# sailist/emotion-recognition-in-conversation

Measured on AMD Instinct MI355X. Metric: utterances/sec training step, COGMEN IEMOCAP-6 atv, higher is better.
Workload: dtype bf16

## Files before the change

emotion-recognition-in-conversation_amd/capi.py:

```python
import ctypes as C
import os
import re
import subprocess

import torch

_HERE = os.path.dirname(os.path.abspath(__file__))
LIB_PATH = os.environ.get("ERC_LIB_PATH") or os.path.join(_HERE, "lib", "libercgraft.so")
CSRC = os.path.join(_HERE, "csrc")
HEADER = os.path.join(os.path.dirname(_HERE), "include", "ercgraft.h")


class ErcGraftError(RuntimeError):
    pass


_CTYPES = {"int": C.c_int, "int32_t": C.c_int, "int64_t": C.c_int64, "uint64_t": C.c_uint64, "float": C.c_float}


def _ctype(decl, proto, ret=False):
    t = " ".join(decl.replace("*", " * ").split())
    if ret and t == "const char *":
        return C.c_char_p
    if "*" in t:
# ... 940 lines not shown
        _call("erc_dgcn_tail", *args)
    else:
        _call("erc_dgcn_tail_cap", *args, n_dev, label_rows)


def dgcn_tail_eval(slabs, n_slabs, slab_stride, rgcn_bias, g, window, W_rel, b_rel, W_root, W1, b1, W2, b2, labels, n_classes,
                   n_rows, Xc, ldx, cm, logits=None, n_dev=None, label_rows=None):
    if cm.dtype != torch.int64 or cm.numel() != n_classes * n_classes or not cm.is_contiguous():
        raise ErcGraftError("dgcn_tail_eval: cm must be a contiguous int64 [%d, %d] tensor" % (n_classes, n_classes))
    _call("erc_dgcn_tail_eval", slabs, n_slabs, int(slab_stride), rgcn_bias, g["in_ptr"], g["in_src"], window, W_rel, b_rel, W_root,
          W1, b1, W2, b2, labels, label_rows, n_classes, n_rows, n_dev, Xc, ldx, cm, logits)


def head_ce_stats_floats(n_rows):
    return int(lib().erc_head_ce_stats_floats(n_rows))


def head_ce(Z, ldz, F, Cn, n_rows, W, bias, labels, weight, mask_scale, logits, ldl, dlogits, lddl, dZ, lddz, stats, n_dev=None):
    args = (Z, ldz, F, Cn, n_rows, W, bias, labels, weight, float(mask_scale), logits, ldl, dlogits, lddl, dZ, lddz, stats)
    if n_dev is None:
        _call("erc_head_ce", *args)
    else:
        _call("erc_head_ce_cap", *args, n_dev)


def cim_meta(lengths, B, T, n_cap, node_off, node_row):
    _call("erc_cim_meta", lengths, B, T, n_cap, node_off, node_row)


def gru_scan_fwd(GX, W_hhT, b_hh, lengths, node_off, B, T, rows, Hout, Hdrop, drop_p, rng, rng_stream, gates, ghn, Hprev):
    _call("erc_gru_scan_fwd", GX, W_hhT, b_hh, lengths, node_off, B, T, rows, Hout, Hdrop, drop_p, rng, rng_stream, gates, ghn,
          Hprev)


def gru_scan_bwd(W_hh, lengths, node_off, B, T, rows, gates, ghn, Hprev, dH, drop_p, rng, rng_stream, dGX, dGH):
    _call("erc_gru_scan_bwd", W_hh, lengths, node_off, B, T, rows, gates, ghn, Hprev, dH, drop_p, rng, rng_stream, dGX, dGH)


def cim_max_t():
    return int(lib().erc_cim_max_t())


def cim_attn_fwd(merged, node_off, B, T, Pbuf):
    _call("erc_cim_attn_fwd", merged, node_off, B, T, Pbuf)


def cim_attn_bwd(merged, dmerged, node_off, B, T, Pbuf, mask_scale):
    _call("erc_cim_attn_bwd", merged, dmerged, node_off, B, T, Pbuf, mask_scale)


def ce_bce_multitask(logits, ld, Cn, n_rows, labels, emo_label, lde, w_ce, w_bce, grad_scale, dlogits, lddl, stats):
    if labels.dtype != torch.int64 or emo_label.dtype != torch.int64:
        raise ErcGraftError("ce_bce_multitask: label and emo_label must be int64")
    if labels.numel() < n_rows or emo_label.dim() != 2 or emo_label.shape[0] < n_rows or emo_label.shape[1] < 7 \
            or emo_label.stride(1) != 1 or logits.numel() < (n_rows - 1) * ld + Cn + 7:
        raise ErcGraftError("ce_bce_multitask: operands smaller than %d rows (label %s, emo_label %s)"
                            % (n_rows, tuple(labels.shape), tuple(emo_label.shape)))
    _call("erc_ce_bce_multitask", logits, ld, Cn, n_rows, labels, emo_label, lde, w_ce, w_bce, grad_scale, dlogits, lddl,
          stats)


def dgcnv2_max_t():
    return int(lib().erc_dgcnv2_max_t())


def dgcnv2_meta(onehot, S, lengths, B, T, n_cap, spk, node_row):
    _call("erc_dgcnv2_meta", onehot, S, lengths, B, T, n_cap, spk, node_row)


def dgcnv2_edge_att_fwd(S, ldS, g, B, T, wp, wf, norm):
    _call("erc_dgcnv2_edge_att_fwd", S, ldS, g["node_off"], B, T, wp, wf, g["out_ptr"], g["out_dst"], g["out_eid"], norm)


def dgcnv2_edge_att_bwd(S, ldS, g, B, T, wp, wf, dnorm, dS, dn_parts=1, dn_stride=0):
    _call("erc_dgcnv2_edge_att_bwd", S, ldS, g["node_off"], B, T, wp, wf, g["out_ptr"], g["out_dst"], g["out_eid"], dnorm,
          dn_parts, dn_stride, dS)


def match_att_fwd(E, lde, Q, ldq, node_off, B, T, F, A, lda, P, TH):
    _call("erc_match_att_fwd", E, lde, Q, ldq, node_off, B, T, F, A, lda, P, TH)


def match_att_bwd(E, lde, Q, ldq, dA, ldda, node_off, B, T, F, P, TH, DZ, dQ, lddq, dE, ldde, n_cap=0):
    args = (E, lde, Q, ldq, dA, ldda, node_off, B, T, F, P, TH, DZ, dQ, lddq, dE, ldde)
    if n_cap:
        _call("erc_match_att_bwd_cap", *args, n_cap)
    else:
        _call("erc_match_att_bwd", *args)


DIALOGRNN_SAVE = {"gates_g": (0, 450), "ghn_g": (450, 150), "g_prev": (600, 150), "g": (750, 150), "g_drop": (900, 150),
                  "c": (1050, 150), "gates_p": (1200, 450), "ghn_p": (1650, 150), "q_prev": (1800, 150), "q": (1950, 150),
                  "q_drop": (2100, 150), "gates_e": (2250, 300), "ghn_e": (2550, 100), "e_prev": (2650, 100), "e": (2750, 100),
                  "e_drop": (2850, 100)}
DIALOGRNN_DREC = {"dgh_g": (0, 450), "dgh_p": (450, 450), "dgi_e": (900, 300), "dgh_e": (1200, 300)}
DIALOGRNN_DREC_ROW = 1500
DIALOGRNN_GXW = 1050


def dialogrnn_max_t():
    return int(lib().erc_dialogrnn_max_t())


def dialogrnn_wt_floats():
    return int(lib().erc_dialogrnn_wt_floats())


def dialogrnn_save_floats(N, B, T):
    return int(lib().erc_dialogrnn_save_floats(N, B, T))


def dialogrnn_planes(buf, N, layout):
    return {k: buf[o * 2 * N:(o + w) * 2 * N].view(2, N, w) for k, (o, w) in layout.items()}


def dialogrnn_alpha(save, N, B, T):
    o = 2950 * 2 * N
    return save[o:o + 2 * B * T * T].view(2, B, T, T)


def dialogrnn_offsets(offs):
    if len(offs) != 20:
        raise ErcGraftError("dialogrnn: 20 parameter offsets expected, got %d" % len(offs))
    return (C.c_int64 * 20)(*[int(o) for o in offs])


def dialogrnn_meta(onehot, S, lengths, B, T, n_cap, node_off, node_row, node_spk):
    _call("erc_dialogrnn_meta", onehot, S, lengths, B, T, n_cap, node_off, node_row, node_spk)


def dialogrnn_pack(params, offs, D_m, WT):
    _call("erc_dialogrnn_pack", params, C.addressof(offs), D_m, WT)


def dialogrnn_scan_fwd(GX, ldgx, WT, params, offs, D_m, node_off, node_spk, B, T, S, N, drop_p, drop_rec, rng, rng_stream,
                       emotions, lde, save):
    _call("erc_dialogrnn_scan_fwd", GX, ldgx, WT, params, C.addressof(offs), D_m, node_off, node_spk, B, T, S, N, float(drop_p),
          float(drop_rec), rng, rng_stream, emotions, lde, save)


def dialogrnn_scan_bwd(GX, ldgx, WT, params, offs, D_m, node_off, node_spk, B, T, S, N, drop_p, drop_rec, rng, rng_stream, save,
                       dEmo, ldde, dGX, lddgx, dREC):
    _call("erc_dialogrnn_scan_bwd", GX, ldgx, WT, params, C.addressof(offs), D_m, node_off, node_spk, B, T, S, N, float(drop_p),
          float(drop_rec), rng, rng_stream, save, dEmo, ldde, dGX, lddgx, dREC)


def bcrnn_meta_cap(lengths, desc, store_label, zero_store_row, B, T, n_cap, node_off, node_row, pad_node, x_row, label_out, counts):
    _call("erc_bcrnn_meta_cap", lengths, desc, store_label, zero_store_row, B, T, n_cap, node_off, node_row, pad_node, x_row,
          label_out, counts)


def log_softmax_rows(x, ldx, Cn, n_rows, y, ldy):
    _call("erc_log_softmax_rows", x, ldx, Cn, n_rows, y, ldy)
```

emotion-recognition-in-conversation_amd/engine.py:

```python
import math
import os

import torch

from . import capi

ALIGN = 64


class WorkspaceCache:

    def __init__(self, maxsize=None):
        import collections
        self.maxsize = int(os.environ.get("ERC_WS_CACHE", 4)) if maxsize is None else maxsize
        self._d = collections.OrderedDict()
        self.last = None

    def get(self, key, make):
        ws = self._d.get(key)
        if ws is None:
            ws = make()
            self._d[key] = ws
            while len(self._d) > self.maxsize:
                victim = next((k for k in self._d if k != key), None)
# ... 410 lines not shown
        dev = flat.device
        self.state = torch.zeros(4 + 512, dtype=torch.int64, device=dev)
        self.state[2] = seed
        self.gnorm = torch.zeros(1, dtype=torch.float32, device=dev)
        self.norm_ws = torch.zeros(1024, dtype=torch.float32, device=dev)
        self.shadow = None
        self.shadow_table = None
        self.skip_flag = None

    def set_step(self, step):
        self.state[0] = int(step)
        self.state[4:] = int(step)

    @property
    def rng_state(self):
        return self.state[1:3]

    def enable_p2p(self, group=None):
        import torch.distributed as dist
        if os.environ.get("ERC_DP_P2P", "0") != "1" or not (dist.is_available() and dist.is_initialized()) or \
                dist.get_world_size(group) < 2 or self.clip_norm > 0 or self.flat.numel > P2PExchange.MAX_PARAMS:
            return False
        try:
            self.flat.p2p = P2PExchange(self.flat, group)
        except P2PUnavailable as exc:
            import sys
            print("ERC_DP_P2P=1: %s -- keeping the RCCL all-reduce" % exc, file=sys.stderr)
            return False
        self.skip_flag = self.flat.health
        return True

    def step(self, grad_scale=1.0):
        f = self.flat
        if getattr(f, "p2p", None) is not None:
            capi.adam_step_p2p(f.data, f.grad, f.exp_avg, f.exp_avg_sq, f.numel, self.lr, self.betas[0], self.betas[1], self.eps,
                               self.weight_decay, self.decoupled, grad_scale, self.state, self.shadow_table, f.p2p.desc)
            return
        if self.clip_norm > 0:
            capi.grad_norm(f.grad, f.numel, grad_scale, self.gnorm, self.norm_ws)
        if self.shadow_table is not None:
            capi.adam_step_tab(f.data, f.grad, f.exp_avg, f.exp_avg_sq, f.numel, self.lr, self.betas[0], self.betas[1],
                               self.eps, self.weight_decay, self.decoupled, grad_scale, self.clip_norm,
                               self.gnorm if self.clip_norm > 0 else None, self.state, self.shadow_table,
                               skip_flag=self.skip_flag)
            return
        capi.adam_step(f.data, f.grad, f.exp_avg, f.exp_avg_sq, f.numel, self.lr, self.betas[0], self.betas[1],
                       self.eps, self.weight_decay, self.decoupled, grad_scale, self.clip_norm,
                       self.gnorm if self.clip_norm > 0 else None, self.state,
                       *(self.shadow if self.shadow is not None else (None, 0, 0)), skip_flag=self.skip_flag)


class P2PUnavailable(RuntimeError):
    """the fused gradient exchange cannot be set up on this node (every rank raises it together)"""


class P2PExchange:

    MAX_PARAMS = 512 * 1024

    def __init__(self, flat, group=None):
        import ctypes as C
        import torch.distributed as dist
        self.world, self.rank = dist.get_world_size(group), dist.get_rank(group)
        if self.world > 8 or flat.numel > self.MAX_PARAMS or flat.numel % 4:
            raise capi.ErcGraftError("P2P gradient exchange: world <= 8 and <= %d parameters (this module: %d)" % (
                self.MAX_PARAMS, flat.numel))
        self.n_pad = flat.numel
        self._mine, self._peers = [], []
        try:
            self._mine = [capi.p2p_alloc(2 * self.n_pad * 4), capi.p2p_alloc(self.world * 512 * 4)]
            mine = (self._mine[0][1], self._mine[1][1])
        except capi.ErcGraftError as exc:
            mine = None
            self.alloc_error = str(exc)
        handles = [None] * self.world
        dist.all_gather_object(handles, mine, group=group)
        if any(h is None for h in handles):
            self.close()
            raise P2PUnavailable("rank(s) %s could not allocate uncached peer-visible memory" % [r for r, h in enumerate(handles) if h is None])
        self.allocation = "hipDeviceMallocUncached"
        x = capi.ErcP2P()
        x.world, x.rank, x.spin_limit, x.n_pad = self.world, self.rank, int(os.environ.get("ERC_P2P_SPIN", 0)), self.n_pad
        for r in range(self.world):
            if r == self.rank:
                x.pub[r], x.flags[r] = self._mine[0][0], self._mine[1][0]
            else:
                pp, pf = capi.p2p_open(handles[r][0]), capi.p2p_open(handles[r][1])
                self._peers += [pp, pf]
                x.pub[r], x.flags[r] = pp, pf
        self.epoch = torch.zeros(512, dtype=torch.int64, device=flat.device)
        x.epoch, x.health = self.epoch.data_ptr(), flat.health.data_ptr()
        self.desc, self.flat = x, flat
        dist.barrier(group=group)

    def close(self):
        for p in self._peers:
            capi.p2p_close(p)
        self._peers = []
        for p, _ in self._mine:
            capi.p2p_free(p)
        self._mine = []


def all_reduce_grads(flat, always=False):
    import torch.distributed as dist
    if dist.is_available() and dist.is_initialized() and (dist.get_world_size() > 1 or always):
        if getattr(flat, "p2p", None) is not None:
            return 1.0 / dist.get_world_size()
        dist.all_reduce(flat.grad_full)
        return 1.0 / dist.get_world_size()
    return 1.0


class SideStream:

    def __init__(self, enabled=None):
        if enabled is None:
            import os
            enabled = os.environ.get("ERC_SIDE_STREAM", "0") == "1"
        self.enabled = enabled and torch.cuda.is_available()
        self.stream = torch.cuda.Stream() if self.enabled else None
        self._dirty = False

    def fork(self):
        return _Fork(self)

    def join(self):
        if self.enabled and self._dirty:
            ev = torch.cuda.Event()
            ev.record(self.stream)
            torch.cuda.current_stream().wait_event(ev)
            self._dirty = False


class _Fork:
    def __init__(self, side):
        self.side = side

    def __enter__(self):
        if self.side.enabled:
            ev = torch.cuda.Event()
            ev.record()
            self.side.stream.wait_event(ev)
            self.ctx = torch.cuda.stream(self.side.stream)
            self.ctx.__enter__()
            self.side._dirty = True

    def __exit__(self, *exc):
        if self.side.enabled:
            self.ctx.__exit__(*exc)
        return False


class GraphedStep:

    def __init__(self, fn, warmup=2, steps=1):
        self.fn = fn
        side = torch.cuda.Stream()
        side.wait_stream(torch.cuda.current_stream())
        with torch.cuda.stream(side):
            for _ in range(warmup):
                self.out = fn()
        torch.cuda.current_stream().wait_stream(side)
        torch.cuda.synchronize()
        self.graph = torch.cuda.CUDAGraph()
        with torch.cuda.graph(self.graph):
            for _ in range(steps):
                self.out = fn()
        self.warmup_steps, self.steps = warmup, steps

    def __call__(self):
        self.graph.replay()
        return self.out
```

emotion-recognition-in-conversation_amd/trainer.py:

```python
import contextlib
import dataclasses
import json
import os
import sys
import time

import numpy as np
import torch
from torch.utils.data import DataLoader

from . import capi
from .capacity import node_capacity
from .collate import ERCCollate
from .synthetic import make_dialogues, make_mosei_dialogues


def fix_seed(seed):
    import random
    random.seed(seed)
    np.random.seed(seed)
    torch.manual_seed(seed)
    if torch.cuda.is_available():
        torch.cuda.manual_seed_all(seed)


class ListDataset(torch.utils.data.Dataset):

    def __init__(self, dialogs):
        self.dialogs = dialogs

    def __len__(self):
        return len(self.dialogs)

    def __getitem__(self, i):
        return [self.dialogs[i]]


class StoreLoader:

    def __init__(self, store, batch_size, shuffle, seed):
        self.store, self.batch_size, self.shuffle = store, batch_size, shuffle
        self.gen = torch.Generator().manual_seed(seed)

    def __len__(self):
        return -(-len(self.store) // self.batch_size)

    def __iter__(self):
        n = len(self.store)
        order = torch.randperm(n, generator=self.gen) if self.shuffle else torch.arange(n)
        for i in range(0, n, self.batch_size):
            yield self.store.batch(order[i:i + self.batch_size])


def shard_dialogues(dialogs, rank, world):
    n = len(dialogs)
    if world <= 1 or n == 0:
        return list(dialogs)
    total = -(-n // world) * world
    idx = [i % n for i in range(total)]
    return [dialogs[i] for i in idx[rank::world]]


def load_dialogues(params, rank=0, world=1):
    if not params.get("synthetic", True):
        from .datasets import read_dialogues
        roots = params.get("data_root", None)
        train = read_dialogues(params.dataset, "train", roots)
        return shard_dialogues(train, rank, world), read_dialogues(params.dataset, "test", roots)
    meld, mosei = "meld" in params.dataset, "mosei" in params.dataset
    lo, hi = (1, 33) if meld else (1, 98) if mosei else (20, 110)
    lo, hi = int(params.get("syn_min_len", lo)), int(params.get("syn_max_len", hi))
    if mosei:
        mk = lambda n, seed: make_mosei_dialogues(n, params.dims(), min_len=lo, max_len=hi, seed=seed)
        return mk(params.n_train, params.seed + 1000 * rank), mk(params.n_test, params.seed + 7)
    mk = lambda n, seed: make_dialogues(n, params.dims(), n_speakers=params.n_speakers, n_classes=params.n_classes,
                                        min_len=lo, max_len=hi, seed=seed)
    return mk(params.n_train, params.seed + 1000 * rank), mk(params.n_test, params.seed + 7)


def make_loaders(params, rank=0, world=1, device=None):
    train_d, test_d = load_dialogues(params, rank, world)
    if params.get("device_collate", False):
        from .datasets import DeviceDialogueStore
        dt = torch.bfloat16 if params.compute == "bf16" else torch.float32
        return (StoreLoader(DeviceDialogueStore(train_d, params, device, dt), params.train.batch_size, True, params.seed + rank),
                StoreLoader(DeviceDialogueStore(test_d, params, device, dt), params.test.batch_size, False, 0))
    train, test = ListDataset(train_d), ListDataset(test_d)
    collate = ERCCollate(params)
    gen = torch.Generator().manual_seed(params.seed + rank)
    tl = DataLoader(train, batch_size=params.train.batch_size, shuffle=True, collate_fn=collate,
                    num_workers=params.train.get("num_workers", 0) or 0, generator=gen)
    el = DataLoader(test, batch_size=params.test.batch_size, shuffle=False, collate_fn=collate, num_workers=0)
    return tl, el


def longest_dialogue(loader):
    if isinstance(loader, StoreLoader):
        return int(loader.store.lengths.max())
    return max(len(d["label"]) for d in loader.dataset.dialogs)


def bucket_t_cap(loader, world, device):
    t = longest_dialogue(loader)
    if world > 1:
        import torch.distributed as dist
        v = torch.tensor([t], dtype=torch.int64, device=device)
        dist.all_reduce(v, op=dist.ReduceOp.MAX)
        t = int(v.item())
    return t


def first_batch(loader):
    if isinstance(loader, StoreLoader):
        return loader.store.batch(torch.arange(min(loader.batch_size, len(loader.store))))
    n = min(loader.batch_size, len(loader.dataset))
    return loader.collate_fn([loader.dataset[i] for i in range(n)])


class FixedBatches:

    def __init__(self, loader, trainer, seed):
        self.batches = [(int(b["label"].shape[0]), trainer.prepare_batch(b)) for b in loader]
        self.gen = torch.Generator().manual_seed(seed)

    def __len__(self):
        return len(self.batches)

    def __iter__(self):
        for i in torch.randperm(len(self.batches), generator=self.gen).tolist():
            yield i, self.batches[i]


def batch_table(lengths, offsets, order, B):
    n = len(order)
    steps = -(-n // B)
    flat = np.zeros((2, steps * B), dtype=np.int32)
    flat[0, :n], flat[1, :n] = lengths[order], offsets[order]
    return np.concatenate([flat[0].reshape(steps, B), flat[1].reshape(steps, B)], axis=1)


@contextlib.contextmanager
def dynamic_n(model, on=True):
    if on:
        model.dynamic_n = True
    try:
        yield
    finally:
        if on:
            model.dynamic_n = False


@dataclasses.dataclass
class GraphEntry:
    static: dict
    fill: object
    capacity: bool
    seen: int = 0
    graph: object = None
    out: object = None
    workspace: object = None


class StepGraphs:

    def __init__(self, trainer, maxsize=16, capture=True):
        import collections
        self.trainer, self.maxsize = trainer, maxsize
        self.capture = capture
        self.cache = collections.OrderedDict()
        self.replays = self.eager = self.captures = 0
        self.capture_failed = False
        self.lazy = True

    def _capture(self, fn):
        torch.cuda.synchronize()
        g = torch.cuda.CUDAGraph()
        with torch.cuda.graph(g):
            out = fn()
        return g, out

    def _sync(self):
        torch.cuda.synchronize()

    @staticmethod
    def shape_key(batch):
        return tuple((k, tuple(v.shape), str(v.dtype)) for k, v in sorted(batch.items()) if torch.is_tensor(v)) + \
            tuple((k, v) for k, v in sorted(batch.items()) if isinstance(v, int))

    @staticmethod
    def _copy_in(static, batch):
        for k, v in batch.items():
            if torch.is_tensor(v):
                static[k].copy_(v, non_blocking=True)

    def _eager_then_capture(self, ent, capture=True, must=False):
        tr = self.trainer
        with dynamic_n(tr.model, ent.capacity):
            stats = tr.train_step(ent.static)
            if not capture:
                return stats
            try:
                ent.graph, ent.out = self._capture(lambda: tr.train_step(ent.static))
            except Exception as exc:
                if must:
                    raise
                print(json.dumps({"graph_replay": "capture failed, staying eager", "error": str(exc)[:200]}), file=sys.stderr)
                self.capture_failed = True
                return stats
        ent.workspace = getattr(tr.model, "_last_ws", None)
        self.captures += 1
        return stats

    def precapture(self, probe):
        tr = self.trainer
        flat, model = tr.model.flat, tr.model
        opt = getattr(tr, "optim", None)
        saved = {k: v.clone() for k, v in model.state_dict().items() if "running_" in k or "num_batches" in k}
        snap = [(t, t.clone()) for t in (getattr(flat, n, None) for n in ("data", "exp_avg", "exp_avg_sq", "grad_full")) if t is not None]
        if opt is not None and getattr(opt, "state", None) is not None:
            snap.append((opt.state, opt.state.clone()))
        if getattr(flat, "p2p", None) is not None:
            snap.append((flat.p2p.epoch, flat.p2p.epoch.clone()))
        for key, make, fill, synth in tr.all_capacity_buckets(probe):
            ent = self.cache[key] = GraphEntry(make(), fill, True, seen=1)
            synth(ent.static)
            self._eager_then_capture(ent, must=True)
        self._sync()
        with torch.no_grad():
            for t, keep in snap:
                t.copy_(keep)
            sd = model.state_dict()
            for k, v in saved.items():
                sd[k].copy_(v)
        flat.health.zero_()
        flat.events.zero_()
        if getattr(model, "shadows", None) is not None:
            model.refresh_shadows()
        self.maxsize = max(self.maxsize, len(self.cache) + 2)

    def step(self, batch, key=None, resident=False):
        bucket = None
        if key is not None:
            key = (key, )
        else:
            bucket = self.trainer.capacity_bucket(batch) if hasattr(self.trainer, "capacity_bucket") else None
            key = bucket[0] if bucket is not None else self.shape_key(batch)
        ent = self.cache.get(key)
        if ent is None and not self.lazy:
            self.eager += 1
            return self.trainer.train_step(batch)
        if ent is None:
            if bucket is not None:
                static, fill = bucket[1](), bucket[2]
            else:
                static = batch if resident else {k: (v.clone() if torch.is_tensor(v) else v) for k, v in batch.items()}
                fill = None if resident else self._copy_in
            ent = self.cache[key] = GraphEntry(static, fill, bucket is not None)
            while len(self.cache) > self.maxsize:
                self.cache.popitem(last=False)
        else:
            self.cache.move_to_end(key)
        ent.seen += 1
        if ent.fill is not None and (ent.graph is not None or ent.seen > 1 or ent.capacity):
            ent.fill(ent.static, batch)
        if ent.graph is not None:
            self.replays += 1
            ent.graph.replay()
            return ent.out
        self.eager += 1
        return self._eager_then_capture(ent, capture=self.capture and not self.capture_failed and
                                        (ent.capacity or ent.seen >= 2 or resident))


class ResidentLoop:

    N_BUCKET = 128

    def __init__(self, trainer, store, batch_size, capture=True):
        self.trainer, self.store, self.B = trainer, store, int(batch_size)
        self.T = int(store.lengths.max())
        named = getattr(trainer, "RESIDENT_N_BUCKET", None)
        if named:
            self.N_BUCKET = max(1, min(int(named), self.B * self.T))
        self.cur_desc = torch.zeros(2 * self.B, dtype=torch.int32, device=store.device)
        self.graphs, self.capture = {}, capture
        self.replays = self.eager = self.captures = 0

    def _capture(self, fn):
        torch.cuda.synchronize()
        g = torch.cuda.CUDAGraph()
        with torch.cuda.graph(g):
            fn()
        return g

    def _caps_of(self, counts):
        return [node_capacity(c, self.N_BUCKET, self.B * self.T) for c in counts]

    def _visit(self, cap):
        ent = self.graphs.get(cap)
        batch = ent[1] if ent is not None else self._batch(cap)
        if batch is None:
            raise capi.ErcGraftError("%s: the trainer offers no resident batch of capacity %d" % (type(self).__name__, cap))
        ws = self._step(batch)
        self.eager += 1
        graph = None
        if self.capture:
            graph = self._capture(lambda: self._step(batch))
            self.captures += 1
        self.graphs[cap] = (graph, batch, ws)

    def _steps(self, table_dev, caps):
        cur_desc, graphs = self.cur_desc, self.graphs
        for s, cap in enumerate(caps):
            cur_desc.copy_(table_dev[s], non_blocking=True)
            ent = graphs.get(cap)
            if ent is not None and ent[0] is not None:
                ent[0].replay()
                self.replays += 1
                continue
            self._visit(cap)


class ResidentEpochs(ResidentLoop):

    def __init__(self, trainer, store, batch_size, seed, capture=True):
        super().__init__(trainer, store, batch_size, capture)
        self.gen = torch.Generator().manual_seed(seed)
        self.acc = torch.zeros(4, dtype=torch.float64, device=store.device)
        self._lens32, self._offs32 = store.lengths.to(torch.int32).numpy(), store.offsets[:-1].to(torch.int32).numpy()
        self._ahead = []

    def plan(self, n_epochs):
        n, B = len(self.store), self.B
        tabs = np.zeros((n_epochs, -(-n // B), 2 * B), dtype=np.int32)
        for e in range(n_epochs):
            tabs[e] = batch_table(self._lens32, self._offs32, torch.randperm(n, generator=self.gen).numpy(), B)
        dev = torch.from_numpy(tabs).to(self.store.device)
        for e in range(n_epochs):
            counts = tabs[e, :, :B].sum(1).tolist()
            self._ahead.append((sum(counts), self._caps_of(counts), dev[e]))

    def supported(self):
        lens = sorted((int(v) for v in self.store.lengths.tolist()), reverse=True)
        worst = self._caps_of([sum(lens[:self.B])])[0]
        return all(self._batch(cap) is not None for cap in sorted({self.N_BUCKET, max(worst, self.N_BUCKET)}))

    def _batch(self, cap):
        return self.trainer.resident_batch(self.store, self.cur_desc, self.B, self.T, cap)

    def _step(self, batch):
        self.acc.add_(self.trainer.train_step(batch)[:4])
        return getattr(self.trainer.model, "_last_ws", None)

    def epoch(self):
        if not self._ahead:
            self.plan(1)
        n_utt, caps, table_dev = self._ahead.pop(0)
        with dynamic_n(self.trainer.model):
            self._steps(table_dev, caps)
        return n_utt, len(caps)


class ResidentEval(ResidentLoop):

    def __init__(self, trainer, store, batch_size, capture=True, n_classes=None):
        super().__init__(trainer, store, batch_size, capture)
        self.table = batch_table(store.lengths.to(torch.int32).numpy(), store.offsets[:-1].to(torch.int32).numpy(),
                                 np.arange(len(store)), self.B)
        self.steps = len(self.table)
        self.counts = self.table[:, :self.B].sum(1).tolist()
        self.caps = self._caps_of(self.counts)
        self.table_dev = torch.from_numpy(self.table).to(store.device)
        C = int(n_classes if n_classes is not None else trainer.params.n_classes)
        self.cm = torch.zeros(C, C, dtype=torch.int64, device=store.device)

    def supported(self):
        return all(self._batch(cap) is not None for cap in sorted(set(self.caps)))

    def _batch(self, cap):
        return self.trainer.resident_eval_batch(self.store, self.cur_desc, self.B, self.T, cap)

    def _step(self, batch):
        return self.trainer.resident_eval_step(batch, self.cm)

    def epoch(self):
        self.cm.zero_()
        self._steps(self.table_dev, self.caps)
        return self.cm.cpu()


def report_from_cm(cm):
    cm = np.asarray(cm, dtype=np.int64)
    n = int(cm.sum())
    tp, sup, prd = np.diag(cm).astype(np.float64), cm.sum(1).astype(np.float64), cm.sum(0).astype(np.float64)
    div = lambda a, b: np.divide(a, b, out=np.zeros_like(a), where=b > 0)
    rec, pre, f1 = div(tp, sup), div(tp, prd), div(2.0 * tp, sup + prd)
    weighted = lambda v: float((v * sup).sum() / n) if n else 0.0
    acc = float(tp.sum() / n) if n else 0.0
    seen = (sup > 0) | (prd > 0)
    return {
        "cm": cm.tolist(),
        "acc": acc,
        "wa": float(rec[sup > 0].mean()) if n else 0.0,
        "pre": weighted(pre),
        "rec": weighted(rec),
        "f1": weighted(f1),
        "mif1": acc,
        "maf1": float(f1[seen].mean()) if n else 0.0,
    }


def classification_report(true, pred, n_classes):
    from sklearn import metrics
    return {
        "cm": metrics.confusion_matrix(true, pred, labels=range(n_classes)).tolist(),
        "acc": metrics.accuracy_score(true, pred),
        "wa": metrics.balanced_accuracy_score(true, pred),
        "pre": metrics.precision_score(true, pred, average="weighted", zero_division=0),
        "rec": metrics.recall_score(true, pred, average="weighted", zero_division=0),
        "f1": metrics.f1_score(true, pred, average="weighted", zero_division=0),
        "mif1": metrics.f1_score(true, pred, average="micro", zero_division=0),
        "maf1": metrics.f1_score(true, pred, average="macro", zero_division=0),
    }


def weighted_accuracy(y_true, y_pred):
    y_true, y_pred = np.asarray(y_true), np.asarray(y_pred)
    P = int((y_true == 1).sum())
    N = len(y_true) - P
    if P == 0 or N == 0:
        return None
    TP = int(((y_true == 1) & (y_pred == 1)).sum())
    TN = int(((y_true == 0) & (y_pred == 0)).sum())
    return (1.0 * TP * (N / (1.0 * P)) + TN) / (2.0 * N)


def multiemo_report(true_multi, prob_multi, thresh=0.5):
    from sklearn import metrics
    true_multi, pred = np.asarray(true_multi), (np.asarray(prob_multi) > thresh).astype(int)
    acc, f1, wa = [], [], []
    for i in range(true_multi.shape[1]):
        col = pred[:, i]
        acc.append(float(metrics.accuracy_score(true_multi[:, i], col)))
        f1.append(float(metrics.precision_recall_fscore_support(true_multi[:, i], col, average="weighted", zero_division=0)[2]))
        wa.append(weighted_accuracy(true_multi[:, i], col))
    defined = [w for w in wa if w is not None]
# ... 192 lines not shown
```

include/ercgraft.h:

```cpp
#ifndef ERCGRAFT_H
#define ERCGRAFT_H

#include <stdint.h>

#ifdef __cplusplus
extern "C" {
#endif

#define ERC_ABI_VERSION 3

#define ERC_OK 0
#define ERC_E_ARG (-1)
#define ERC_E_LAUNCH (-2)

int erc_abi_version(void);
const char* erc_last_error(void);

int erc_window_graph_build(const int64_t* lengths, const int64_t* speakers, int64_t spk_sb, int64_t spk_st,
                           int B, int T, int wp, int wf, int n_speakers, int n_cap, int e_cap,
                           int32_t* node_off, int32_t* node_row, int32_t* node_spk,
                           int32_t* in_ptr, int32_t* in_src, int32_t* in_typ,
                           int32_t* out_ptr, int32_t* out_dst, int32_t* out_typ, int32_t* out_eid,
                           int64_t* edge_index, int64_t* edge_type, int32_t* counts, void* stream);
int erc_window_graph_build_desc(const int64_t* lengths, const int64_t* speakers, int64_t spk_sb, int64_t spk_st,
// ... 404 lines not shown
int erc_transpose_batched(const float* in, int nb, int rows, int cols, float* out, void* stream);
int erc_csr_sum(const float* x, int ldx, int F, int N, const int32_t* ptr, const int32_t* idx, float* out, int ldo,
                int accumulate, void* stream);

int erc_dgcn_tail_max_rows(void);
int erc_dgcn_tail_set_stamps(uint64_t* stamps);
int erc_dgcn_tail_max_window(void);
int64_t erc_dgcn_tail_stats_floats(int n_rows);
int erc_dgcn_tail(const float* slabs, int n_slabs, int64_t slab_stride, const float* rgcn_bias, const int32_t* in_ptr,
                  const int32_t* in_src, int window, const float* W_rel, const float* b_rel, const float* W_root,
                  const float* W1, const float* b1, const float* W2, const float* b2, const int64_t* labels,
                  const float* weight, int n_classes, int n_rows, float drop_p, const uint64_t* rng, float* Xc, int ldx,
                  float* Hc, float* AGG, float* Zc, float* logits, float* dlogits, float* dZc, float* dXc, int lddx,
                  float* dAGG, float* dHc, float* stats, void* stream);
int erc_dgcn_tail_cap(const float* slabs, int n_slabs, int64_t slab_stride, const float* rgcn_bias, const int32_t* in_ptr,
                      const int32_t* in_src, int window, const float* W_rel, const float* b_rel, const float* W_root,
                      const float* W1, const float* b1, const float* W2, const float* b2, const int64_t* labels,
                      const float* weight, int n_classes, int n_rows, float drop_p, const uint64_t* rng, float* Xc, int ldx,
                      float* Hc, float* AGG, float* Zc, float* logits, float* dlogits, float* dZc, float* dXc, int lddx,
                      float* dAGG, float* dHc, float* stats, const int32_t* n_dev, const int32_t* label_rows, void* stream);

int erc_dgcn_tail_eval(const float* slabs, int n_slabs, int64_t slab_stride, const float* rgcn_bias, const int32_t* in_ptr,
                       const int32_t* in_src, int window, const float* W_rel, const float* b_rel, const float* W_root,
                       const float* W1, const float* b1, const float* W2, const float* b2, const int64_t* labels,
                       const int32_t* label_rows, int n_classes, int n_rows, const int32_t* n_dev, const float* Xc, int ldx,
                       int64_t* cm, float* logits, void* stream);

int erc_gemm_f32_grouped(int form, const float* A, int lda, const float* B, int ldb, float* C, int ldc,
                         int N_or_K, const int32_t* node_off, int n_dialogues, int n_mod, int n_nodes,
                         int max_len, int pitch, int accumulate, int act, const float* aux, int ldaux,
                         float act_scale,
                         const float* cross, int planes, int64_t a_plane, int64_t b_plane, int split, int64_t c_slab,
                         void* stream);
int erc_gemm_f32_planes(const float* A, int lda, int64_t a_plane, const float* B, int ldb, int64_t b_plane, float* C,
                        int ldc, int M, int N, int K, int planes, int split_k, int64_t c_slab, int accumulate,
                        void* stream);
int erc_mm_meta(const int64_t* lengths, const float* qmask, int64_t q_st, int64_t q_sb, int n_speakers, int B,
                int32_t* node_off, int32_t* node_row, int32_t* node_dlg, int32_t* node_spk, void* stream);
int erc_mm_flatten(const float* src, int lds, const int32_t* row_map, const float* emb, const int32_t* spk, int N,
                   float* dst, int ldd, void* stream);
int64_t erc_mm_emb_grad_ws_floats(int n_speakers);
int erc_mm_emb_grad(const float* dl, int ld, const int32_t* spk, int N, int n_speakers, float* demb, float* ws,
                    void* stream);
int erc_mm_row_normalize(const float* x, int R, float* xhat, float* inv, void* stream);
int erc_mm_row_normalize_bwd(const float* xhat, const float* inv, const float* dxhat, int R, float* dx, void* stream);
int erc_mm_adj_finish(const float* COS, const float* xhat, const int32_t* node_off, int B, int M, int N, int P,
                      float* ADJ, float* CR, float* CCOS, float* DEG, void* stream);
int erc_mm_adj_finish_bwd(const float* COS, const float* CCOS, const float* DEG, const float* dADJ, const float* dCR,
                          const int32_t* node_off, int B, int M, int N, int P, float* G, float* GC, float* DD,
                          void* stream);
int erc_mm_cross_apply(const float* CR, const float* h, int ldh, const int32_t* node_dlg, const int32_t* node_off,
                       int M, int N, int P, float* out, int ldo, void* stream);
int erc_mm_cross_grad(const float* dhi, int ldd, const float* h, int ldh, const int32_t* node_dlg,
                      const int32_t* node_off, int M, int N, int P, float* dCR, int planes, int64_t d_plane,
                      int64_t h_plane, void* stream);
int erc_gcnii_combine_fwd(const float* G, const float* hi, const float* h0, int64_t n, float theta, float alpha,
                          float drop_p, const uint64_t* rng_state, uint64_t rng_stream, float* hd, void* stream);
int erc_gcnii_combine_bwd(const float* d_hd, const float* hd, int64_t n, float theta, float alpha, float keep_scale,
                          int plain, float* dG, float* dhi, float* dh0, int F, int ld_d, void* stream);
int erc_gcnii_layer_fwd(const float* hih0, int lda, const float* W, int ldw, float theta, float alpha, float drop_p,
                        const uint64_t* rng_state, uint64_t rng_stream, float* hd, int ldo, int rows, int F, void* stream);
int erc_dropout_fwd(const float* x, int64_t n, float drop_p, const uint64_t* rng_state, uint64_t rng_stream, float* y,
                    void* stream);
int erc_mm_regroup_fwd(const float* xd, const float* hl, int M, int N, float drop_p, const uint64_t* rng_state,
                       uint64_t rng_stream, float* FE, void* stream);
int erc_mm_regroup_bwd(const float* dFE, const float* FE, int M, int N, float keep_scale, float* d_xd, float* d_h,
                       void* stream);
int erc_axpy_mask(const float* x, const float* mask, int64_t n, float scale, int accumulate, float* y, void* stream);
int erc_mm_meta_cap(const int64_t* lengths, const float* qmask, int64_t q_st, int64_t q_sb, int n_speakers, const int32_t* desc,
                    const int64_t* store_spk, const int64_t* store_label, int zero_store_row, int B, int T, int n_cap,
                    int32_t* node_off, int32_t* node_row, int32_t* node_pad, int32_t* node_dlg, int32_t* node_spk,
                    int32_t* pad_node, int32_t* x_row, int64_t* label_out, int32_t* counts, void* stream);
int erc_mm_flatten_cap(const float* src, int lds, const int32_t* row_map, const float* emb, const int32_t* spk, int n_cap,
                       const int32_t* n_dev, float* dst, int ldd, void* stream);
int erc_mm_emb_grad_cap(const float* dl, int ld, const int32_t* spk, int n_cap, const int32_t* n_dev, int n_speakers, float* demb,
                        float* ws, void* stream);
int erc_mm_row_normalize_cap(const float* x, int n_mod, int n_cap, const int32_t* n_dev, float* xhat, float* inv, void* stream);
int erc_mm_row_normalize_bwd_cap(const float* xhat, const float* inv, const float* dxhat, int n_mod, int n_cap,
                                 const int32_t* n_dev, float* dx, void* stream);
int erc_mm_cross_apply_cap(const float* CR, const float* h, int ldh, const int32_t* node_dlg, const int32_t* node_off, int M,
                           int n_cap, const int32_t* n_dev, int P, float* out, int ldo, void* stream);
int erc_mm_cross_grad_cap(const float* dhi, int ldd, const float* h, int ldh, const int32_t* node_dlg, const int32_t* node_off,
                          int M, int n_cap, const int32_t* n_dev, int P, float* dCR, int planes, int64_t d_plane,
                          int64_t h_plane, void* stream);
int erc_gcnii_combine_bwd_cap(const float* d_hd, const float* hd, int n_mod, int n_cap, const int32_t* n_dev, float theta,
                              float alpha, float keep_scale, int plain, float* dG, float* dhi, float* dh0, int F, int ld_d,
                              void* stream);
int erc_dropout_fwd_cap(const float* x, int n_mod, int n_cap, const int32_t* n_dev, int row_w, float drop_p,
                        const uint64_t* rng_state, uint64_t rng_stream, float* y, void* stream);
int erc_mm_regroup_fwd_cap(const float* xd, const float* hl, int M, int n_cap, const int32_t* n_dev, float drop_p,
                           const uint64_t* rng_state, uint64_t rng_stream, float* FE, void* stream);
int erc_mm_regroup_bwd_cap(const float* dFE, const float* FE, int M, int n_cap, const int32_t* n_dev, float keep_scale,
                           float* d_xd, float* d_h, void* stream);
int erc_axpy_mask_cap(const float* x, const float* mask, int n_mod, int n_cap, const int32_t* n_dev, int row_w, float scale,
                      int accumulate, float* y, void* stream);
int erc_mm_zero_tail(float* buf, int64_t ld, int width, int n_mod, int n_cap, const int32_t* n_dev, void* stream);


int erc_cim_meta(const int64_t* lengths, int B, int T, int n_cap, int32_t* node_off, int32_t* node_row, void* stream);
int erc_gru_scan_fwd(const float* GX, const float* W_hhT, const float* b_hh, const int64_t* lengths, const int32_t* node_off,
                     int B, int T, int64_t rows, float* Hout, float* Hdrop, float drop_p, const uint64_t* rng_state,
                     uint64_t rng_stream, float* gates, float* ghn, float* Hprev, void* stream);
int erc_gru_scan_bwd(const float* W_hh, const int64_t* lengths, const int32_t* node_off, int B, int T, int64_t rows,
                     const float* gates, const float* ghn, const float* Hprev, const float* dH, float drop_p,
                     const uint64_t* rng_state, uint64_t rng_stream, float* dGX, float* dGH, void* stream);
int erc_cim_max_t(void);
int erc_cim_attn_fwd(float* merged, const int32_t* node_off, int B, int T, float* Pbuf, void* stream);
int erc_cim_attn_bwd(const float* merged, float* dmerged, const int32_t* node_off, int B, int T, const float* Pbuf,
                     float mask_scale, void* stream);
int erc_ce_bce_multitask(const float* logits, int ld, int C, int n_rows, const int64_t* label, const int64_t* emo_label,
                         int lde, float w_ce, float w_bce, float grad_scale, float* dlogits, int lddl, float* stats,
                         void* stream);

int erc_dgcnv2_max_t(void);
int erc_dgcnv2_meta(const float* onehot, int S, const int64_t* lengths, int B, int T, int n_cap, int64_t* spk,
                    int32_t* node_row, void* stream);
int erc_dgcnv2_edge_att_fwd(const float* S, int ldS, const int32_t* node_off, int B, int T, int wp, int wf,
                            const int32_t* out_ptr, const int32_t* out_dst, const int32_t* out_eid, float* norm, void* stream);
int erc_dgcnv2_edge_att_bwd(const float* S, int ldS, const int32_t* node_off, int B, int T, int wp, int wf,
                            const int32_t* out_ptr, const int32_t* out_dst, const int32_t* out_eid, const float* dnorm,
                            int dn_parts, int64_t dn_stride, float* dS, void* stream);


int erc_match_att_fwd(const float* E, int lde, const float* Q, int ldq, const int32_t* node_off, int B, int T, int F, float* A,
                      int lda, float* P, float* TH, void* stream);
int erc_match_att_bwd(const float* E, int lde, const float* Q, int ldq, const float* dA, int ldda, const int32_t* node_off,
                      int B, int T, int F, const float* P, const float* TH, float* DZ, float* dQ, int lddq, float* dE, int ldde,
                      void* stream);
int erc_match_att_bwd_cap(const float* E, int lde, const float* Q, int ldq, const float* dA, int ldda, const int32_t* node_off,
                          int B, int T, int F, const float* P, const float* TH, float* DZ, float* dQ, int lddq, float* dE,
                          int ldde, int n_cap, void* stream);


int erc_dialogrnn_max_t(void);
int64_t erc_dialogrnn_wt_floats(void);
int64_t erc_dialogrnn_save_floats(int64_t N, int B, int T);
int erc_dialogrnn_meta(const float* onehot, int S, const int64_t* lengths, int B, int T, int n_cap, int32_t* node_off,
                       int32_t* node_row, int32_t* node_spk, void* stream);
int erc_dialogrnn_pack(const float* params, const int64_t* offs_host, int D_m, float* WT, void* stream);
int erc_dialogrnn_scan_fwd(const float* GX, int ldgx, const float* WT, const float* params, const int64_t* offs_host, int D_m,
                           const int32_t* node_off, const int32_t* node_spk, int B, int T, int S, int64_t N, float drop_p,
                           float drop_rec, const uint64_t* rng_state, uint64_t rng_stream, float* emotions, int lde,
                           float* save, void* stream);
int erc_dialogrnn_scan_bwd(const float* GX, int ldgx, const float* WT, const float* params, const int64_t* offs_host, int D_m,
                           const int32_t* node_off, const int32_t* node_spk, int B, int T, int S, int64_t N, float drop_p,
                           float drop_rec, const uint64_t* rng_state, uint64_t rng_stream, const float* save,
                           const float* dEmo, int ldde, float* dGX, int lddgx, float* dREC, void* stream);
int erc_bcrnn_meta_cap(const int64_t* lengths, const int32_t* desc, const int64_t* store_label, int zero_store_row, int B, int T,
                       int n_cap, int32_t* node_off, int32_t* node_row, int32_t* pad_node, int32_t* x_row, int64_t* label_out,
                       int32_t* counts, void* stream);
int erc_log_softmax_rows(const float* x, int ldx, int C, int n_rows, float* y, int ldy, void* stream);


int erc_test_poison_lds(int32_t* sink, void* stream);

#ifdef __cplusplus
}
#endif
#endif
```

Measured before the change: 21.38 million.

## Replay captured training steps as direct kernel launches instead of HIP graph replay

Adds a HIP-side chain builder that reads a captured step graph, checks that it is a single linear path of this library's kernel nodes, and records each node's function, grid, block, shared-memory size and argument pointers. In the default auto mode, captured steps then replay by issuing those kernels with hipLaunchKernel in order, and fall back to hipGraph replay when the graph does not qualify. The intent is to avoid HIP graph launch overhead in a launch-bound training step. In exchange, it keeps the raw graph alive so the argument pointers stay valid, pays host-side per-kernel launch cost, and only applies to purely linear graphs.

```diff
diff --git a/emotion-recognition-in-conversation_amd/capi.py b/emotion-recognition-in-conversation_amd/capi.py
--- a/emotion-recognition-in-conversation_amd/capi.py
+++ b/emotion-recognition-in-conversation_amd/capi.py
@@ -1116,3 +1116,31 @@
 
 def log_softmax_rows(x, ldx, Cn, n_rows, y, ldy):
     _call("erc_log_softmax_rows", x, ldx, Cn, n_rows, y, ldy)
+
+
+def chain_order(n_nodes, edges):
+    ne = len(edges)
+    fr, to = (C.c_int32 * max(1, ne))(*[e[0] for e in edges]), (C.c_int32 * max(1, ne))(*[e[1] for e in edges])
+    order = (C.c_int32 * max(1, n_nodes))()
+    _call("erc_chain_order", n_nodes, ne, C.addressof(fr), C.addressof(to), C.addressof(order))
+    return list(order)[:n_nodes]
+
+
+def chain_build(raw_graph):
+    handle = int(lib().erc_chain_build(raw_graph))
+    return (handle, None) if handle else (0, lib().erc_last_error().decode())
+
+
+def chain_len(chain):
+    n = int(lib().erc_chain_len(chain))
+    if n < 0:
+        _check(n, "erc_chain_len")
+    return n
+
+
+def chain_run(chain):
+    _check(lib().erc_chain_run(chain, stream()), "erc_chain_run")
+
+
+def chain_free(chain):
+    _check(lib().erc_chain_free(chain), "erc_chain_free")
diff --git a/emotion-recognition-in-conversation_amd/csrc/launch_chain.hip b/emotion-recognition-in-conversation_amd/csrc/launch_chain.hip
--- /dev/null
+++ b/emotion-recognition-in-conversation_amd/csrc/launch_chain.hip
@@ -0,0 +1,144 @@
+#include <dlfcn.h>
+
+#include <vector>
+
+#include "erc_common.h"
+
+extern "C" int erc_chain_order(int n_nodes, int n_edges, const int32_t* from_host, const int32_t* to_host, int32_t* order_host) {
+    ERC_REQUIRE(n_nodes > 0 && order_host != nullptr, "chain_order: n_nodes=%d (need >= 1 and an output array)", n_nodes);
+    ERC_REQUIRE(n_edges == n_nodes - 1, "chain_order: %d nodes with %d edges are not one path", n_nodes, n_edges);
+    ERC_REQUIRE(n_edges == 0 || (from_host != nullptr && to_host != nullptr), "chain_order: null edge list");
+    std::vector<int32_t> next(n_nodes, -1), pred(n_nodes, -1);
+    for (int e = 0; e < n_edges; ++e) {
+        const int32_t a = from_host[e], b = to_host[e];
+        ERC_REQUIRE(a >= 0 && a < n_nodes && b >= 0 && b < n_nodes && a != b, "chain_order: edge %d (%d -> %d) out of range", e, a, b);
+        ERC_REQUIRE(next[a] < 0, "chain_order: node %d has two successors (a fork)", a);
+        ERC_REQUIRE(pred[b] < 0, "chain_order: node %d has two predecessors (a join)", b);
+        next[a] = b;
+        pred[b] = a;
+    }
+    int root = -1, roots = 0;
+    for (int i = 0; i < n_nodes; ++i)
+        if (pred[i] < 0) {
+            root = i;
+            ++roots;
+        }
+    ERC_REQUIRE(roots == 1, "chain_order: %d roots (need exactly one)", roots);
+    int len = 0;
+    for (int i = root; i >= 0 && len < n_nodes; i = next[i]) order_host[len++] = i;
+    ERC_REQUIRE(len == n_nodes, "chain_order: only %d of %d nodes hang on the root's path", len, n_nodes);
+    return ERC_OK;
+}
+
+namespace {
+
+constexpr uint32_t CHAIN_MAGIC = 0x45524343u;
+
+struct ChainNode {
+    const void* func;
+    dim3 grid, block;
+    unsigned lds;
+    void** params;
+};
+
+struct Chain {
+    uint32_t magic;
+    std::vector<ChainNode> nodes;
+};
+
+Chain* chain_of(int64_t handle) {
+    Chain* c = reinterpret_cast<Chain*>(static_cast<intptr_t>(handle));
+    return (c != nullptr && c->magic == CHAIN_MAGIC) ? c : nullptr;
+}
+
+Chain* refuse(const char* what, hipError_t e) {
+    erc_set_error("chain_build: %s%s%s", what, e != hipSuccess ? ": " : "", e != hipSuccess ? hipGetErrorString(e) : "");
+    (void)hipGetLastError();
+    return nullptr;
+}
+
+Chain* build(hipGraph_t graph) {
+    if (graph == nullptr) return refuse("null graph", hipSuccess);
+    size_t n = 0, n_edges = 0;
+    hipError_t e = hipGraphGetNodes(graph, nullptr, &n);
+    if (e != hipSuccess) return refuse("hipGraphGetNodes", e);
+    if (n == 0 || n > (1u << 20)) return refuse("the graph has no nodes (or too many)", hipSuccess);
+    std::vector<hipGraphNode_t> nodes(n);
+    if ((e = hipGraphGetNodes(graph, nodes.data(), &n)) != hipSuccess) return refuse("hipGraphGetNodes", e);
+    nodes.resize(n);
+    if ((e = hipGraphGetEdges(graph, nullptr, nullptr, &n_edges)) != hipSuccess) return refuse("hipGraphGetEdges", e);
+    if (n_edges != n - 1) return refuse("the nodes do not form one path (edge count)", hipSuccess);
+    std::vector<hipGraphNode_t> from(n_edges + 1), to(n_edges + 1);
+    if (n_edges > 0 && (e = hipGraphGetEdges(graph, from.data(), to.data(), &n_edges)) != hipSuccess) return refuse("hipGraphGetEdges", e);
+    if (n_edges != n - 1) return refuse("the nodes do not form one path (edge count)", hipSuccess);
+
+    std::vector<ChainNode> found(n);
+    for (size_t i = 0; i < n; ++i) {
+        hipGraphNodeType type;
+        if ((e = hipGraphNodeGetType(nodes[i], &type)) != hipSuccess) return refuse("hipGraphNodeGetType", e);
+        if (type != hipGraphNodeTypeKernel) return refuse("a node is not a kernel node (memcpy, memset, host, event ...)", hipSuccess);
+        hipKernelNodeParams p;
+        if ((e = hipGraphKernelNodeGetParams(nodes[i], &p)) != hipSuccess) return refuse("hipGraphKernelNodeGetParams", e);
+        if (p.kernelParams == nullptr || p.extra != nullptr) return refuse("a kernel node passes its arguments through `extra`", hipSuccess);
+        hipFuncAttributes attr;
+        if ((e = hipFuncGetAttributes(&attr, p.func)) != hipSuccess) return refuse("a kernel node's function cannot be launched by host address", e);
+        Dl_info own, theirs;
+        if (dladdr(reinterpret_cast<const void*>(&erc_chain_order), &own) == 0 || dladdr(p.func, &theirs) == 0 ||
+            own.dli_fbase != theirs.dli_fbase)
+            return refuse("a kernel node's function is not one of libercgraft's kernels", hipSuccess);
+        found[i] = ChainNode{p.func, p.gridDim, p.blockDim, p.sharedMemBytes, p.kernelParams};
+    }
+    std::vector<int32_t> fi(n_edges + 1), ti(n_edges + 1), order(n);
+    for (size_t k = 0; k < n_edges; ++k) {
+        int32_t a = -1, b = -1;
+        for (size_t i = 0; i < n; ++i) {
+            if (nodes[i] == from[k]) a = (int32_t)i;
+            if (nodes[i] == to[k]) b = (int32_t)i;
+        }
+        fi[k] = a;
+        ti[k] = b;
+    }
+    if (erc_chain_order((int)n, (int)n_edges, fi.data(), ti.data(), order.data()) != ERC_OK) return nullptr;
+    Chain* c = new Chain{CHAIN_MAGIC, {}};
+    c->nodes.reserve(n);
+    for (size_t i = 0; i < n; ++i) c->nodes.push_back(found[order[i]]);
+    return c;
+}
+
+}
+
+extern "C" int64_t erc_chain_build(void* graph_host) {
+    return static_cast<int64_t>(reinterpret_cast<intptr_t>(build(static_cast<hipGraph_t>(graph_host))));
+}
+
+extern "C" int erc_chain_len(int64_t chain) {
+    Chain* c = chain_of(chain);
+    ERC_REQUIRE(c != nullptr, "chain_len: not a chain handle");
+    return (int)c->nodes.size();
+}
+
+extern "C" int erc_chain_run(int64_t chain, void* stream) {
+    Chain* c = chain_of(chain);
+    ERC_REQUIRE(c != nullptr, "chain_run: not a chain handle");
+    const hipStream_t s = static_cast<hipStream_t>(stream);
+    const size_t n = c->nodes.size();
+    for (size_t i = 0; i < n; ++i) {
+        const ChainNode& k = c->nodes[i];
+        const hipError_t e = hipLaunchKernel(k.func, k.grid, k.block, k.params, k.lds, s);
+        if (e != hipSuccess) {
+            erc_set_error("chain_run: launch %d of %d failed: %s", (int)i, (int)n, hipGetErrorString(e));
+            (void)hipGetLastError();
+            return ERC_E_LAUNCH;
+        }
+    }
+    return ERC_OK;
+}
+
+extern "C" int erc_chain_free(int64_t chain) {
+    if (chain == 0) return ERC_OK;
+    Chain* c = chain_of(chain);
+    ERC_REQUIRE(c != nullptr, "chain_free: not a chain handle");
+    c->magic = 0;
+    delete c;
+    return ERC_OK;
+}
diff --git a/emotion-recognition-in-conversation_amd/engine.py b/emotion-recognition-in-conversation_amd/engine.py
--- a/emotion-recognition-in-conversation_amd/engine.py
+++ b/emotion-recognition-in-conversation_amd/engine.py
@@ -586,6 +586,56 @@
         return False
 
 
+def step_replay_mode():
+    mode = os.environ.get("ERC_STEP_REPLAY", "") or "auto"
+    if mode not in ("auto", "graph", "launches"):
+        raise capi.ErcGraftError("ERC_STEP_REPLAY=%s: expected 'graph' or 'launches'" % mode)
+    return mode
+
+
+class CapturedStep:
+
+    def __init__(self, fn, steps=1, mode=None):
+        self.mode = mode or step_replay_mode()
+        self.chain, self.refused = 0, None
+        keep = self.mode != "graph"
+        self.graph = torch.cuda.CUDAGraph(keep_graph=True) if keep else torch.cuda.CUDAGraph()
+        with torch.cuda.graph(self.graph):
+            for _ in range(steps):
+                self.out = fn()
+        if keep:
+            self.chain, self.refused = capi.chain_build(self.graph.raw_cuda_graph())
+            if not self.chain:
+                if self.mode == "launches":
+                    raise capi.ErcGraftError("ERC_STEP_REPLAY=launches: the captured step cannot be replayed as plain launches: %s"
+                                             % self.refused)
+                self.graph.instantiate()
+        self.launches = capi.chain_len(self.chain) if self.chain else None
+        self._run = capi.lib().erc_chain_run if self.chain else None
+
+    @property
+    def replays_by(self):
+        return "launches" if self.chain else "graph"
+
+    def replay(self):
+        if self.chain:
+            capi._check(self._run(self.chain, torch.cuda.current_stream().cuda_stream), "erc_chain_run")
+        else:
+            self.graph.replay()
+
+    def close(self):
+        chain, self.chain = self.chain, 0
+        if chain:
+            capi.chain_free(chain)
+        self.graph = None
+
+    def __del__(self):
+        try:
+            self.close()
+        except Exception:
+            pass
+
+
 class GraphedStep:
 
     def __init__(self, fn, warmup=2, steps=1):
@@ -597,12 +647,10 @@
                 self.out = fn()
         torch.cuda.current_stream().wait_stream(side)
         torch.cuda.synchronize()
-        self.graph = torch.cuda.CUDAGraph()
-        with torch.cuda.graph(self.graph):
-            for _ in range(steps):
-                self.out = fn()
+        self.captured = CapturedStep(fn, steps=steps)
+        self.out = self.captured.out
         self.warmup_steps, self.steps = warmup, steps
 
     def __call__(self):
-        self.graph.replay()
+        self.captured.replay()
         return self.out
diff --git a/emotion-recognition-in-conversation_amd/trainer.py b/emotion-recognition-in-conversation_amd/trainer.py
--- a/emotion-recognition-in-conversation_amd/trainer.py
+++ b/emotion-recognition-in-conversation_amd/trainer.py
@@ -12,6 +12,7 @@
 from . import capi
 from .capacity import node_capacity
 from .collate import ERCCollate
+from .engine import CapturedStep
 from .synthetic import make_dialogues, make_mosei_dialogues
 
 
@@ -174,10 +175,8 @@
 
     def _capture(self, fn):
         torch.cuda.synchronize()
-        g = torch.cuda.CUDAGraph()
-        with torch.cuda.graph(g):
-            out = fn()
-        return g, out
+        g = CapturedStep(fn)
+        return g, g.out
 
     def _sync(self):
         torch.cuda.synchronize()
@@ -288,10 +287,7 @@
 
     def _capture(self, fn):
         torch.cuda.synchronize()
-        g = torch.cuda.CUDAGraph()
-        with torch.cuda.graph(g):
-            fn()
-        return g
+        return CapturedStep(fn)
 
     def _caps_of(self, counts):
         return [node_capacity(c, self.N_BUCKET, self.B * self.T) for c in counts]
diff --git a/include/ercgraft.h b/include/ercgraft.h
--- a/include/ercgraft.h
+++ b/include/ercgraft.h
@@ -580,6 +580,12 @@
 int erc_log_softmax_rows(const float* x, int ldx, int C, int n_rows, float* y, int ldy, void* stream);
 
 
+int erc_chain_order(int n_nodes, int n_edges, const int32_t* from_host, const int32_t* to_host, int32_t* order_host);
+int64_t erc_chain_build(void* graph_host);
+int erc_chain_len(int64_t chain);
+int erc_chain_run(int64_t chain, void* stream);
+int erc_chain_free(int64_t chain);
+
 int erc_test_poison_lds(int32_t* sink, void* stream);
 
 #ifdef __cplusplus
```

Measured after the change: 22.64 million (median of 6 runs). 1.06x the previous value.
